# als244/ResNet

Hardware: AMD Instinct MI355X
Metric: images/sec ResNet-50 fp32 224x224 batch256 (higher is better)
Workload: dtype f32

## Files before the change

### resnet_amd/csrc/kernels_igemm.hip

```cpp
#include "mi_common.hpp"
#include <type_traits>
#include "mi_device.h"

typedef float f32x16 __attribute__((ext_vector_type(16)));
typedef float pf4 __attribute__((ext_vector_type(4)));

enum { IG_FWD = 0, IG_DGRAD = 1, IG_WGRAD = 2 };

struct IgArgs {
    int N, C, K, H, W, Ho, Wo;
    int HW, P;
    int ncols;
    int mtiles;
    int tiles;
    int ctiles;
    int klen;
    FastDiv fdP, fdWo, fdM;
    int full, tsplit, tklen, cpt;
    FastDiv fdTs, fdCpt;
    float *tailbuf;
    float *bn_part;
    int bn_np;
    const float *bnb_x, *bnb_mask, *bnb_mean;
    float *bnb_part;
// ... 345 lines not shown
        for (; it + 2 < ntiles; it++) kstep(Y, Y, it & 1);
        if (it + 1 < ntiles) { kstep(Y, NO, it & 1); it++; }
        if (it < ntiles) kstep(NO, NO, it & 1);
    }

    IG_T(2);
    if (MODE != IG_WGRAD && tail_id >= 0) {
        float *tb = g.tailbuf + (size_t)tail_id * (BM * 128);
#pragma unroll
        for (int j = 0; j < TN; j++)
#pragma unroll
            for (int i = 0; i < 2; i++)
#pragma unroll
                for (int r = 0; r < 16; r++)
                    tb[(wm * 64 + i * 32 + (r & 3) + 8 * (r >> 2) + 4 * (lane >> 5)) * 128 + wn * WNC + j * 32 + (lane & 31)] = acc[i][j][r];
        return;
    }
    if (MODE == IG_DGRAD && S == 1 && g.bnb_part) {
        constexpr int PPT = 4 / WMW;
        if ((g.P & 3) == 0) {
            constexpr int CPR = WNC / 4, RPI = 64 / CPR, PITCH = WNC + 4;
            float *img = ig_smem + wave * (32 * PITCH);
            const int c4 = (lane % CPR) * 4, r0 = lane / CPR;
            const int col = n0 + wn * WNC + c4;
            const bool cok = col < g.ncols;
            const uint32_t jc = cok ? (uint32_t)col : 0u;
            const uint32_t nimg = fd_div(jc, g.fdP);
            const size_t coff = (size_t)nimg * g.C * g.HW + (jc - nimg * g.P);
            const size_t pplane = (size_t)g.bnb_np * g.C;
#pragma unroll
            for (int i = 0; i < 2; i++) {
#pragma unroll
                for (int j = 0; j < TN; j++)
#pragma unroll
                    for (int r = 0; r < 16; r++)
                        img[((r & 3) + 8 * (r >> 2) + 4 * (lane >> 5)) * PITCH + j * 32 + (lane & 31)] = acc[i][j][r];
#pragma unroll
                for (int ps = 0; ps < 32 / RPI; ps++) {
                    const int rl = ps * RPI + r0;
                    const int row = m0 + wm * 64 + i * 32 + rl;
                    const size_t o = coff + (size_t)row * g.HW;
                    const pf4 z = {0.f, 0.f, 0.f, 0.f};
                    pf4 v = *(const pf4 *)(img + rl * PITCH + c4);
                    pf4 xv = z, mv = z;
                    if (cok) {
                        if (addend) v += *(const pf4 *)(addend + o);
                        xv = *(const pf4 *)(g.bnb_x + o);
                        mv = *(const pf4 *)(g.bnb_mask + o);
                    }
                    const float mean = g.bnb_mean[row];
                    float s1 = 0.f, s2 = 0.f;
#pragma unroll
                    for (int e = 0; e < 4; e++) {
                        v[e] = (cok && mv[e] > 0.f) ? v[e] : 0.f;
                        s1 += v[e];
                        s2 = fmaf(v[e], xv[e] - mean, s2);
                    }
                    if (cok) *(pf4 *)(Out + o) = v;
                    s1 += __int_as_float(__builtin_amdgcn_update_dpp(0, __float_as_int(s1), 0xB1, 0xF, 0xF, true));
                    s2 += __int_as_float(__builtin_amdgcn_update_dpp(0, __float_as_int(s2), 0xB1, 0xF, 0xF, true));
                    s1 += __int_as_float(__builtin_amdgcn_update_dpp(0, __float_as_int(s1), 0x4E, 0xF, 0xF, true));
                    s2 += __int_as_float(__builtin_amdgcn_update_dpp(0, __float_as_int(s2), 0x4E, 0xF, 0xF, true));
                    s1 += __int_as_float(__builtin_amdgcn_update_dpp(0, __float_as_int(s1), 0x141, 0xF, 0xF, true));
                    s2 += __int_as_float(__builtin_amdgcn_update_dpp(0, __float_as_int(s2), 0x141, 0xF, 0xF, true));
                    if (CPR == 16) {
                        s1 += __int_as_float(__builtin_amdgcn_update_dpp(0, __float_as_int(s1), 0x140, 0xF, 0xF, true));
                        s2 += __int_as_float(__builtin_amdgcn_update_dpp(0, __float_as_int(s2), 0x140, 0xF, 0xF, true));
                    }
                    if ((lane % CPR) == 0) {
                        const size_t po = (size_t)(ct * PPT + wn) * g.C + row;
                        g.bnb_part[po] = s1;
                        g.bnb_part[pplane + po] = s2;
                    }
                }
            }
            return;
        }
        size_t coffj[TN];
        bool cokj[TN];
#pragma unroll
        for (int j = 0; j < TN; j++) {
            const int col = n0 + wn * WNC + j * 32 + (lane & 31);
            cokj[j] = col < g.ncols;
            const uint32_t jc = cokj[j] ? (uint32_t)col : 0u;
            const uint32_t n = fd_div(jc, g.fdP);
            coffj[j] = (size_t)n * g.C * g.HW + (jc - n * g.P);
        }
        const size_t rstride = (size_t)g.HW;
        const size_t pplane = (size_t)g.bnb_np * g.C;
#pragma unroll
        for (int i = 0; i < 2; i++) {
            float s1[16], s2[16], mn[16];
#pragma unroll
            for (int r = 0; r < 16; r++) {
                s1[r] = 0.f; s2[r] = 0.f;
                mn[r] = g.bnb_mean[m0 + wm * 64 + i * 32 + (r & 3) + 8 * (r >> 2) + 4 * (lane >> 5)];
            }
#pragma unroll
            for (int j = 0; j < TN; j++) {
                float ad[16], xv[16], mv[16];
#pragma unroll
                for (int r = 0; r < 16; r++) {
                    const size_t o = coffj[j] + (size_t)(m0 + wm * 64 + i * 32 + (r & 3) + 8 * (r >> 2) + 4 * (lane >> 5)) * rstride;
                    ad[r] = (addend && cokj[j]) ? addend[o] : 0.f;
                    xv[r] = cokj[j] ? g.bnb_x[o] : 0.f;
                    mv[r] = cokj[j] ? g.bnb_mask[o] : 0.f;
                }
#pragma unroll
                for (int r = 0; r < 16; r++) {
                    const int row = m0 + wm * 64 + i * 32 + (r & 3) + 8 * (r >> 2) + 4 * (lane >> 5);
                    const float gv = mv[r] > 0.f ? acc[i][j][r] + ad[r] : 0.f;
                    if (cokj[j]) Out[coffj[j] + (size_t)row * rstride] = gv;
                    s1[r] += gv;
                    s2[r] = fmaf(gv, xv[r] - mn[r], s2[r]);
                }
            }
#pragma unroll
            for (int r = 0; r < 16; r++) {
                const float t1 = ig_half_sum32(s1[r]), t2 = ig_half_sum32(s2[r]);
                if ((lane & 31) == 31) {
                    const int row = m0 + wm * 64 + i * 32 + (r & 3) + 8 * (r >> 2) + 4 * (lane >> 5);
                    const size_t po = (size_t)(ct * PPT + wn) * g.C + row;
                    g.bnb_part[po] = t1;
                    g.bnb_part[pplane + po] = t2;
                }
            }
        }
        return;
    }
#pragma unroll
    for (int j = 0; j < TN; j++) {
        const int col = n0 + wn * WNC + j * 32 + (lane & 31);
        size_t coff, rstride;
        bool cok;
        if (MODE == IG_WGRAD) {
            const int lc = wn * WNC + j * 32 + (lane & 31);
            const int tap = CT64 ? wg_t + (lc >> 6) : wg_t;
            cok = tap < T;
            coff = ((size_t)((size_t)wg_split * T + tap) * g.K) * g.C + (CT64 ? (lc & 63) : cblk + lc);
            rstride = (size_t)g.C;
        } else {
            cok = col < g.ncols;
            const uint32_t jc = cok ? (uint32_t)col : 0u;
            const uint32_t n = fd_div(jc, g.fdP);
            const uint32_t p = jc - n * g.P;
            if (MODE == IG_FWD) { coff = (size_t)n * g.K * g.P + p; rstride = (size_t)g.P; }
            else if (S == 1) { coff = (size_t)n * g.C * g.HW + p; rstride = (size_t)g.HW; }
            else {
                const uint32_t a = fd_div(p, g.fdWo), b = p - a * g.Wo;
                coff = (size_t)n * g.C * g.HW + (size_t)(2 * a + ph) * g.W + 2 * b + pw;
                rstride = (size_t)g.HW;
            }
        }
        if (!cok) continue;
#pragma unroll
        for (int i = 0; i < 2; i++) {
            float ad[16];
            if (MODE == IG_DGRAD && addend) {
#pragma unroll
                for (int r = 0; r < 16; r++)
                    ad[r] = addend[coff + (size_t)(m0 + wm * 64 + i * 32 + (r & 3) + 8 * (r >> 2) + 4 * (lane >> 5)) * rstride];
            }
#pragma unroll
            for (int r = 0; r < 16; r++) {
                const int row = m0 + wm * 64 + i * 32 + (r & 3) + 8 * (r >> 2) + 4 * (lane >> 5);
                float v = acc[i][j][r];
                if (MODE == IG_DGRAD && addend) v += ad[r];
                Out[coff + (size_t)row * rstride] = v;
            }
        }
    }

    IG_T(3);
    if (MODE == IG_FWD && g.bn_part) {
        constexpr int PPT = 4 / WMW;
        float *tw = ig_smem + wave * (WNC * 64);
        const int l31 = lane & 31;
#pragma unroll
        for (int j = 0; j < TN; j++) {
            const int col = j * 32 + l31;
#pragma unroll
            for (int i = 0; i < 2; i++)
#pragma unroll
                for (int rg = 0; rg < 4; rg++) {
                    const int row4 = i * 8 + rg * 2 + (lane >> 5);
                    pf4 q4 = {acc[i][j][rg * 4 + 0], acc[i][j][rg * 4 + 1], acc[i][j][rg * 4 + 2], acc[i][j][rg * 4 + 3]};
                    *(pf4 *)(tw + col * 64 + ((row4 ^ (col & 15)) << 2)) = q4;
                }
        }
        const int nv = min(WNC, max(0, g.ncols - (n0 + wn * WNC)));
        const int row = lane;
        const float s0 = tw[(((row >> 2) ^ 0) << 2) + (row & 3)];
        float sd = 0.f, sq = 0.f;
#pragma unroll 8
        for (int c = 0; c < WNC; c++) {
            const float x = tw[c * 64 + ((((row >> 2) ^ (c & 15))) << 2) + (row & 3)];
            const float d = c < nv ? x - s0 : 0.f;
            sd += d;
            sq = fmaf(d, d, sq);
        }
        const float inv = nv > 0 ? 1.0f / (float)nv : 0.f;
        const size_t plane = (size_t)g.bn_np * g.K;
        const size_t o = (size_t)(ct * PPT + wn) * g.K + m0 + wm * 64 + row;
        g.bn_part[o] = (float)nv;
        g.bn_part[plane + o] = nv > 0 ? s0 + sd * inv : 0.f;
        g.bn_part[2 * plane + o] = fmaxf(sq - sd * sd * inv, 0.f);
    }
    IG_T(4);
}

template <int MODE, int BM>
__global__ void __launch_bounds__(256)
igemm_tail_reduce_kernel(float *__restrict__ Out, const float *__restrict__ addend, const IgArgs g) {
    const uint32_t L = (uint32_t)g.full + blockIdx.x;
    const uint32_t ct = fd_div(L, g.fdM);
    const int m0 = (int)(L - ct * g.mtiles) * BM;
    const int col = (int)ct * 128 + (threadIdx.x & 127);
    const bool cok = col < g.ncols;
    const uint32_t jc = cok ? (uint32_t)col : 0u;
    const uint32_t n = fd_div(jc, g.fdP);
    const uint32_t p = jc - n * g.P;
    size_t coff, rstride;
    if (MODE == IG_FWD) { coff = (size_t)n * g.K * g.P + p; rstride = (size_t)g.P; }
    else { coff = (size_t)n * g.C * g.HW + p; rstride = (size_t)g.HW; }
    const int row0 = (int)blockIdx.y * 16 + (int)(threadIdx.x >> 7) * 8;
    const float *tb = g.tailbuf + (size_t)blockIdx.x * g.tsplit * (BM * 128) + (size_t)row0 * 128 + (threadIdx.x & 127);
    float v[8];
#pragma unroll
    for (int i = 0; i < 8; i++) v[i] = 0.f;
    for (int z = 0; z < g.tsplit; z++) {
#pragma unroll
        for (int i = 0; i < 8; i++) v[i] += tb[(size_t)z * (BM * 128) + i * 128];
    }
    if (cok) {
#pragma unroll
        for (int i = 0; i < 8; i++) {
            const size_t o = coff + (size_t)(m0 + row0 + i) * rstride;
            float r = v[i];
            if (MODE == IG_DGRAD && addend) r += addend[o];
            Out[o] = r;
        }
    }
    if (MODE == IG_FWD && g.bn_part) {
        constexpr int PPT = BM == 128 ? 2 : 4;
        const int lane = threadIdx.x & 63, l31 = lane & 31;
        const int c32 = (int)ct * 128 + (int)(threadIdx.x & 127 & ~31);
        const int nv = min(32, max(0, g.ncols - c32));
        const size_t plane = (size_t)g.bn_np * g.K;
#pragma unroll
        for (int i = 0; i < 8; i++) {
            float mj, qj, nj = (float)nv;
            ig_half_stats(v[i], nv, l31, mj, qj);
            int pp = (int)(threadIdx.x & 127) >> 5;
            if (PPT == 2) {
                const float n2 = __shfl_xor(nj, 32, 64), m2o = __shfl_xor(mj, 32, 64), q2 = __shfl_xor(qj, 32, 64);
                if (lane == 0) ig_merge(nj, mj, qj, n2, m2o, q2);
                pp >>= 1;
            }
            if (PPT == 2 ? lane == 0 : l31 == 0) {
                const size_t o = (size_t)(ct * PPT + pp) * g.K + m0 + row0 + i;
                g.bn_part[o] = nj;
                g.bn_part[plane + o] = mj;
                g.bn_part[2 * plane + o] = qj;
            }
        }
    }
}

template <int T>
__global__ void __launch_bounds__(256)
igemm_wt_kernel(const float *__restrict__ w, float *__restrict__ out, int K, int C, int to_tck) {
    __shared__ float tile[32][T * 32 + 1];
    const int k0 = blockIdx.y * 32, c0 = blockIdx.x * 32;
    for (int e = threadIdx.x; e < 32 * T * 32; e += 256) {
        const int kr = e / (T * 32), x = e - kr * (T * 32);
        tile[kr][x] = w[((size_t)(k0 + kr) * C + c0) * T + x];
    }
    __syncthreads();
    for (int e = threadIdx.x; e < T * 32 * 32; e += 256) {
        const int t = e >> 10, u = (e >> 5) & 31, v = e & 31;
        if (to_tck) out[((size_t)t * C + c0 + u) * K + k0 + v] = tile[v][u * T + t];
        else out[((size_t)t * K + k0 + u) * C + c0 + v] = tile[u][v * T + t];
    }
}

__global__ void __launch_bounds__(256)
igemm_wt_all_kernel(const mid_wt_entry *__restrict__ entries, const int *__restrict__ tile_entry) {
    __shared__ float tile[32][9 * 32 + 1];
    const mid_wt_entry E = entries[tile_entry[blockIdx.x]];
    const int tl = (int)blockIdx.x - E.tile0, ctiles = E.C / 32, T = E.T;
    const int c0 = (tl % ctiles) * 32, k0 = (tl / ctiles) * 32, row = T * 32;
    for (int e = threadIdx.x; e < 32 * row; e += 256) {
        const int kr = e / row, x = e - kr * row;
        tile[kr][x] = E.w[((size_t)(k0 + kr) * E.C + c0) * T + x];
    }
    __syncthreads();
    for (int e = threadIdx.x; e < T * 1024; e += 256) {
        const int t = e >> 10, u = (e >> 5) & 31, v = e & 31;
        if (E.fwd) E.fwd[((size_t)t * E.C + c0 + u) * E.K + k0 + v] = tile[v][u * T + t];
        if (E.dgrad) E.dgrad[((size_t)t * E.K + k0 + u) * E.C + c0 + v] = tile[u][v * T + t];
    }
}

template <int T>
__global__ void __launch_bounds__(256)
igemm_wgrad_reduce_kernel(const float *__restrict__ part, float *__restrict__ dw, long KC, int splits) {
    const long i = (long)blockIdx.x * 256 + threadIdx.x;
    if (i >= KC) return;
    float s[T];
#pragma unroll
    for (int t = 0; t < T; t++) s[t] = 0.f;
    constexpr int U = T == 1 ? 8 : 2;
    int z = 0;
    for (; z + U <= splits; z += U) {
        float v[U][T];
#pragma unroll
        for (int u = 0; u < U; u++)
#pragma unroll
            for (int t = 0; t < T; t++) v[u][t] = part[((long)(z + u) * T + t) * KC + i];
#pragma unroll
        for (int u = 0; u < U; u++)
#pragma unroll
            for (int t = 0; t < T; t++) s[t] += v[u][t];
    }
    for (; z < splits; z++)
#pragma unroll
        for (int t = 0; t < T; t++) s[t] += part[((long)z * T + t) * KC + i];
#pragma unroll
    for (int t = 0; t < T; t++) dw[i * T + t] = s[t];
}

template <int T, int G>
__global__ void __launch_bounds__(256)
igemm_wgrad_reduce_g_kernel(const float *__restrict__ part, float *__restrict__ dw, long KC, int splits) {
    constexpr int OPB = 256 / G;
    __shared__ float sh[G][OPB][T];
    const int o = threadIdx.x % OPB, gq = threadIdx.x / OPB;
    const long i = (long)blockIdx.x * OPB + o;
    const int chunk = (splits + G - 1) / G, z0 = gq * chunk, z1 = min(splits, z0 + chunk);
    float s[T];
#pragma unroll
    for (int t = 0; t < T; t++) s[t] = 0.f;
    if (i < KC) {
        constexpr int U = T == 1 ? 8 : 2;
        int z = z0;
        for (; z + U <= z1; z += U) {
            float v[U][T];
#pragma unroll
            for (int u = 0; u < U; u++)
#pragma unroll
                for (int t = 0; t < T; t++) v[u][t] = part[((long)(z + u) * T + t) * KC + i];
#pragma unroll
            for (int u = 0; u < U; u++)
#pragma unroll
                for (int t = 0; t < T; t++) s[t] += v[u][t];
        }
        for (; z < z1; z++)
#pragma unroll
            for (int t = 0; t < T; t++) s[t] += part[((long)z * T + t) * KC + i];
    }
#pragma unroll
    for (int t = 0; t < T; t++) sh[gq][o][t] = s[t];
    __syncthreads();
    if (gq == 0 && i < KC) {
#pragma unroll
        for (int t = 0; t < T; t++) {
            float r = sh[0][o][t];
            for (int q = 1; q < G; q++) r += sh[q][o][t];
            dw[i * T + t] = r;
        }
    }
}
static bool igemm_wgrad_reduce_grouped(long KC, int splits) {
    static int on = -1;
    if (on < 0) { const char *e = getenv("RESNET_MI_WGRAD_REDUCE_G"); on = e ? atoi(e) : 1; }
    return on && splits >= 16 && mi_cdiv(KC, 256) < 1024;
}
static const char *igemm_wgrad_reduce_launch(hipStream_t st, const float *part, float *dw, long KC, int k, int splits) {
    const bool grouped = igemm_wgrad_reduce_grouped(KC, splits);
    if (k == 1) {
        if (grouped) hipLaunchKernelGGL((igemm_wgrad_reduce_g_kernel<1, 8>), dim3(mi_cdiv(KC, 32)), dim3(256), 0, st, part, dw, KC, splits);
        else hipLaunchKernelGGL(igemm_wgrad_reduce_kernel<1>, dim3(mi_cdiv(KC, 256)), dim3(256), 0, st, part, dw, KC, splits);
    } else {
        if (grouped) hipLaunchKernelGGL((igemm_wgrad_reduce_g_kernel<9, 8>), dim3(mi_cdiv(KC, 32)), dim3(256), 0, st, part, dw, KC, splits);
        else hipLaunchKernelGGL(igemm_wgrad_reduce_kernel<9>, dim3(mi_cdiv(KC, 256)), dim3(256), 0, st, part, dw, KC, splits);
    }
    return mi_trace_name("igemm_wgrad_reduce_kernel<k%d,%s>", k == 1 ? 1 : 3, grouped ? "grouped" : "flat");
}

__global__ void __launch_bounds__(256)
igemm_wgrad_reduce_t_kernel(const float *__restrict__ part, float *__restrict__ dw, int K, int C, int splits) {
    const long i = (long)blockIdx.x * 256 + threadIdx.x;
    if (i >= (long)K * C) return;
    float s = 0.f;
    int z = 0;
    for (; z + 8 <= splits; z += 8) {
        float v[8];
#pragma unroll
        for (int u = 0; u < 8; u++) v[u] = part[(long)(z + u) * K * C + i];
#pragma unroll
        for (int u = 0; u < 8; u++) s += v[u];
    }
    for (; z < splits; z++) s += part[(long)z * K * C + i];
    const int c = (int)(i / K), kk = (int)(i - (long)c * K);
    dw[(long)kk * C + c] = s;
}

enum { IGOP_FWD = 0, IGOP_DGRAD = 1, IGOP_WGRAD = 2 };
extern "C" int mi_igemm_supported(int op, int N, int C, int H, int K, int k, int stride) {
    if (!((k == 1 && stride == 1) || (k == 3 && (stride == 1 || stride == 2)))) return 0;
    if (H % stride || H / stride < 2) return 0;
    if ((double)N * C * H * H >= 1073741824.0 || (double)N * K * (H / stride) * (H / stride) >= 1073741824.0) return 0;
    if (op == IGOP_FWD) return C % 32 == 0 && K % 64 == 0;
    if (op == IGOP_DGRAD) return K % 32 == 0 && C % 64 == 0;
    if (C % 128 == 0 && K % 64 == 0) return 1;
    if (k == 3 && C == 64 && K % 64 == 0) return 1;
    return k == 1 && C % 64 == 0 && K % 128 == 0;
}
#define IG_SLOTS 512
#define IG_SLOTS64 768
static int igemm_wgrad_splits(int N, int C, int H, int K, int k, int stride) {
    const int bm = K % 128 == 0 ? 128 : 64;
    const long tiles = (C == 64 && k == 3 ? 5L : (long)k * k * (C / 128)) * (K / bm);
    const long ksteps = ((long)N * (H / stride) * (H / stride) + IG_BK - 1) / IG_BK;
    const long slots = bm == 128 ? IG_SLOTS : IG_SLOTS64;
    int best = 1;
    double best_eff = 0;
    for (int s = 1; s <= 512; s++) {
        if (s > 1 && ksteps / s < 48) break;
        const double waves = (double)tiles * s / slots;
        const double eff = waves / (double)((long)((tiles * s + slots - 1) / slots));
        if (eff > best_eff + 0.02) { best_eff = eff; best = s; }
    }
    return best;
}
static bool igemm_wgrad_swapped(int C, int K, int k) { return k == 1 && C % 128 != 0; }
extern "C" size_t mi_igemm_part_floats(int N, int C, int H, int K, int k, int stride) {
    if (igemm_wgrad_swapped(C, K, k)) return (size_t)igemm_wgrad_splits(N, K, H, C, k, stride) * K * C;
    return (size_t)igemm_wgrad_splits(N, C, H, K, k, stride) * k * k * K * C;
}

#define IG_TAIL_FLOATS ((size_t)IG_SLOTS * 128 * 128)
extern "C" size_t mi_igemm_tail_floats(void) { return IG_TAIL_FLOATS; }
static void igemm_tail_plan(IgArgs &g, int ksteps, float *tailbuf, int bm) {
    const int slots = bm == 128 ? IG_SLOTS : IG_SLOTS64;
    g.full = g.tiles; g.tsplit = 1; g.tklen = ksteps; g.tailbuf = tailbuf;
    g.fdTs = make_fastdiv(1);
    static int on = -1;
    if (on < 0) { const char *e = getenv("RESNET_MI_IGEMM_TAIL"); on = e ? atoi(e) : 1; }
    if (!on || !tailbuf) return;
    const int rem = g.tiles % slots;
    if (rem == 0) return;
    if (rem * 2 > slots) return;
    int s = slots / rem;
    if (s > 16) s = 16;
    while (s > 1 && ksteps / s < 8) s--;
    if (s < 2) return;
    g.tklen = (ksteps + s - 1) / s;
    g.tsplit = (ksteps + g.tklen - 1) / g.tklen;
    g.full = g.tiles - rem;
    g.fdTs = make_fastdiv(g.tsplit);
}

static int igemm_pick_bm(int M, int coltiles, int ksteps, int k) {
    if (M % 128) return 64;
    double best = 0;
    int pick = 128;
    for (int bm = 128; bm >= 64; bm -= 64) {
        const long B = (long)(M / bm) * coltiles;
        const long slots = bm == 128 ? IG_SLOTS : IG_SLOTS64;
        const long rem = B % slots;
        double tail = 0;
        if (rem) {
            int s = (int)(slots / rem);
            if (s > 16) s = 16;
            while (s > 1 && ksteps / s < 8) s--;
            tail = rem * 2 > slots || s < 2 ? 1.0 : 1.0 / s + 0.03;
        }
        const double t = ((double)(B / slots) + tail) * (bm == 128 ? 1.0 : k == 1 ? 0.70 : 0.80);
        if (bm == 128 || t < best * 0.97) { if (bm == 128 || t < best) { best = t; pick = bm; } }
    }
    static int force = -1;
    if (force < 0) { const char *e = getenv("RESNET_MI_IGEMM_BM"); force = e ? atoi(e) : 0; }
    if (force == 64 || (force == 128 && M % 128 == 0)) return force;
    return pick;
}

static void igemm_geometry(IgArgs &g, int N, int C, int H, int K, int stride) {
    g.N = N; g.C = C; g.K = K; g.H = H; g.W = H; g.Ho = H / stride; g.Wo = H / stride;
    g.HW = H * H; g.P = g.Ho * g.Wo;
    g.ncols = N * g.P;
    g.fdP = make_fastdiv(g.P); g.fdWo = make_fastdiv(g.Wo);
}
static int igemm_plan_tiles(IgArgs &g, int op, int N, int C, int H, int K, int k, int stride) {
    igemm_geometry(g, N, C, H, K, stride);
    const int M = op == IGOP_FWD ? K : C, red = op == IGOP_FWD ? C : K;
    const int bm = (op == IGOP_FWD || stride == 1) ? igemm_pick_bm(M, mi_cdiv(g.ncols, 128), k * k * (red / IG_BK), k) : (M % 128 == 0 ? 128 : 64);
    g.mtiles = M / bm;
    g.tiles = g.mtiles * mi_cdiv(g.ncols, 128);
    g.fdM = make_fastdiv(g.mtiles);
    g.cpt = red / IG_BK; g.fdCpt = make_fastdiv(g.cpt);
    return bm;
}
static int igemm_plan_wgrad(IgArgs &g, int N, int C, int H, int K, int k, int stride, bool swapped, int *used) {
    int bm;
    if (swapped) {
        const int splits = igemm_wgrad_splits(N, K, H, C, 1, 1);
        igemm_geometry(g, N,  K, H,  C, 1);
        bm = C % 128 == 0 ? 128 : 64;
        g.mtiles = C / bm;
        g.ctiles = K / 128;
        g.tiles = g.mtiles * g.ctiles;
        g.klen = mi_cdiv(mi_cdiv(N * g.P, splits), IG_BK) * IG_BK;
    } else {
        const int T = k * k;
        const int splits = igemm_wgrad_splits(N, C, H, K, k, stride);
        igemm_geometry(g, N, C, H, K, stride);
        bm = K % 128 == 0 ? 128 : 64;
        g.mtiles = K / bm;
        g.ctiles = C / 128;
        g.tiles = C == 64 ? g.mtiles * ((T + 1) / 2) : g.mtiles * T * g.ctiles;
        g.klen = mi_cdiv(mi_cdiv(N * g.P, splits), IG_BK) * IG_BK;
    }
    g.fdM = make_fastdiv(g.mtiles);
    g.full = g.tiles; g.tsplit = 1; g.fdTs = make_fastdiv(1); g.cpt = 1; g.fdCpt = make_fastdiv(1);
    *used = mi_cdiv(N * g.P, g.klen);
    return bm;
}
static thread_local const char *ig_variant = "igemm_kernel";
template <int MODE, int KS, int S, int WMW, bool VB = false>
static int igemm_launch_t(hipStream_t st, dim3 grid, const float *A, const float *B, float *out, const float *addend, const IgArgs &g) {
    constexpr int BM = 64 * WMW;
    constexpr int LDA = (MODE == IG_WGRAD) ? BM + 1 : BM + 4, LDB = (MODE == IG_WGRAD) ? 129 : 132;
    constexpr size_t lds = (size_t)2 * IG_BK * (LDA + LDB) * sizeof(float);
    static int attr_set = 0;
    if (!attr_set) {
        if (lds > 64 * 1024 &&
            hipFuncSetAttribute((const void *)igemm_kernel<MODE, KS, S, WMW, VB>, hipFuncAttributeMaxDynamicSharedMemorySize, (int)lds) != hipSuccess) {
            mi_record_error("igemm_kernel", "cannot raise the dynamic LDS limit");
            return -1;
        }
        attr_set = 1;
    }
    hipLaunchKernelGGL((igemm_kernel<MODE, KS, S, WMW, VB>), grid, dim3(256), lds, st, A, B, out, addend, g);
    ig_variant = mi_trace_name("igemm_kernel<%s,k%d,s%d,bm%d%s%s>", MODE == IG_FWD ? "fwd" : MODE == IG_DGRAD ? "dgrad" : "wgrad", KS, S, BM, VB ? ",vb" : "",
                               g.tsplit > 1 ? ",tail" : "");
    return 0;
}
template <int MODE>
static int igemm_launch(hipStream_t st, dim3 grid, const float *A, const float *B, float *out, const float *addend, const IgArgs &g,
                        int k, int stride, int bm) {
#define IGL(KS_, S_)                                                                                      \
    if (k == KS_ && stride == S_)                                                                         \
        return bm == 128 ? igemm_launch_t<MODE, KS_, S_, 2>(st, grid, A, B, out, addend, g)               \
                         : igemm_launch_t<MODE, KS_, S_, 1>(st, grid, A, B, out, addend, g);
    if (MODE != IG_WGRAD && k == 1 && stride == 1 && g.P % 4 == 0)
        return bm == 128 ? igemm_launch_t<MODE, 1, 1, 2, true>(st, grid, A, B, out, addend, g)
                         : igemm_launch_t<MODE, 1, 1, 1, true>(st, grid, A, B, out, addend, g);
    if (MODE == IG_WGRAD && k == 3 && g.C == 64) {
        if (stride == 1) return bm == 128 ? igemm_launch_t<MODE, 3, 1, 2, true>(st, grid, A, B, out, addend, g) : igemm_launch_t<MODE, 3, 1, 1, true>(st, grid, A, B, out, addend, g);
        return bm == 128 ? igemm_launch_t<MODE, 3, 2, 2, true>(st, grid, A, B, out, addend, g) : igemm_launch_t<MODE, 3, 2, 1, true>(st, grid, A, B, out, addend, g);
    }
    IGL(1, 1) IGL(3, 1) IGL(3, 2)
#undef IGL
    return -2;
}
static int igemm_fam(int k) { return k == 1 ? MI_FAM_GEMM : MI_FAM_PCONV; }

extern "C" int mi_igemm_fwd(mid_stream s, mid_workspace *ws, const float *x, const float *w, float *y, int N, int C, int H, int K, int k,
                            int stride, mid_bn_parts *parts) {
    hipStream_t st = (hipStream_t)s;
    const int T = k * k;
    if (parts) parts->nparts = 0;
    if (!mi_igemm_supported(IGOP_FWD, N, C, H, K, k, stride)) { mi_record_error("mi_igemm_fwd", "shape not supported by the implicit GEMM"); return -2; }
    if (!ws || ws->wt_floats < (size_t)T * C * K) { mi_record_error("mi_igemm_fwd", "workspace too small"); return -3; }
    const float *A = ws->pre_fwd;
    if (!A) {
        if (k == 1) hipLaunchKernelGGL(igemm_wt_kernel<1>, dim3(C / 32, K / 32), dim3(256), 0, st, w, ws->wt, K, C, 1);
        else hipLaunchKernelGGL(igemm_wt_kernel<9>, dim3(C / 32, K / 32), dim3(256), 0, st, w, ws->wt, K, C, 1);
        MI_LAUNCH_CHECK("igemm_wt_kernel");
        A = ws->wt;
    }
    IgArgs g = {};
    const int bm = igemm_plan_tiles(g, IGOP_FWD, N, C, H, K, k, stride);
    igemm_tail_plan(g, T * g.cpt, ws->wt_floats >= (size_t)T * C * K + IG_TAIL_FLOATS ? ws->wt + (size_t)T * C * K : nullptr, bm);
    if (parts) {
        parts->nparts = 0;
        const int np = mi_cdiv(g.ncols, 128) * (bm == 128 ? 2 : 4);
        if (parts->buf && parts->floats >= (size_t)3 * np * K) { g.bn_part = parts->buf; g.bn_np = np; parts->nparts = np; }
    }
    mi_prof_begin(st, igemm_fam(k), 2.0 * T * (double)g.ncols * C * K,
                  4.0 * ((double)N * C * g.HW + (double)T * C * K + (double)g.ncols * K));
    int rc = igemm_launch<IG_FWD>(st, dim3(g.full + (g.tiles - g.full) * g.tsplit), A, x, y, nullptr, g, k, stride, bm);
    if (!rc && g.tsplit > 1) {
        if (bm == 128) hipLaunchKernelGGL((igemm_tail_reduce_kernel<IG_FWD, 128>), dim3(g.tiles - g.full, 8), dim3(256), 0, st, y, nullptr, g);
        else hipLaunchKernelGGL((igemm_tail_reduce_kernel<IG_FWD, 64>), dim3(g.tiles - g.full, 4), dim3(256), 0, st, y, nullptr, g);
    }
    mi_prof_end(st);
    if (rc) return rc;
    MI_LAUNCH_CHECK(ig_variant);
    return 0;
}

extern "C" int mi_igemm_dgrad(mid_stream s, mid_workspace *ws, const float *w, const float *dy, float *dx, const float *addend, int N,
                              int C, int H, int K, int k, int stride, mid_bn_bwd_parts *fz) {
    hipStream_t st = (hipStream_t)s;
    if (fz) fz->nparts = 0;
    if (!mi_igemm_supported(IGOP_DGRAD, N, C, H, K, k, stride)) { mi_record_error("mi_igemm_dgrad", "shape not supported by the implicit GEMM"); return -2; }
    const int T = k * k;
    const float *A = w;
    if (k == 3) {
        if (!ws || ws->wt_floats < (size_t)T * C * K) { mi_record_error("mi_igemm_dgrad", "workspace too small"); return -3; }
        if (ws->pre_dgrad) A = ws->pre_dgrad;
        else {
            hipLaunchKernelGGL(igemm_wt_kernel<9>, dim3(C / 32, K / 32), dim3(256), 0, st, w, ws->wt, K, C, 0);
            MI_LAUNCH_CHECK("igemm_wt_kernel");
            A = ws->wt;
        }
    }
    IgArgs g = {};
    const int bm = igemm_plan_tiles(g, IGOP_DGRAD, N, C, H, K, k, stride);
    bool fused = false;
    if (fz && fz->buf && stride == 1) {
        const int np = mi_cdiv(g.ncols, 128) * (bm == 128 ? 2 : 4);
        if (fz->floats >= (size_t)2 * np * C) {
            g.bnb_x = (const float *)fz->x; g.bnb_mask = (const float *)fz->mask; g.bnb_mean = fz->means;
            g.bnb_part = fz->buf; g.bnb_np = np; fz->nparts = np;
            fused = true;
        }
    }
    igemm_tail_plan(g, T * g.cpt, !fused && stride == 1 && ws && ws->wt_floats >= (size_t)T * C * K + IG_TAIL_FLOATS ? ws->wt + (size_t)T * C * K : nullptr, bm);
    mi_prof_begin(st, igemm_fam(k), 2.0 * T * (double)g.ncols * C * K,
                  4.0 * ((double)g.ncols * K + (double)T * C * K + (double)N * C * g.HW * ((addend ? 2 : 1) + (fused ? 2 : 0))));
    int rc = igemm_launch<IG_DGRAD>(st, dim3(g.full + (g.tiles - g.full) * g.tsplit, stride == 2 ? 4 : 1), A, dy, dx, addend, g, k, stride, bm);
    if (!rc && g.tsplit > 1) {
        if (bm == 128) hipLaunchKernelGGL((igemm_tail_reduce_kernel<IG_DGRAD, 128>), dim3(g.tiles - g.full, 8), dim3(256), 0, st, dx, addend, g);
        else hipLaunchKernelGGL((igemm_tail_reduce_kernel<IG_DGRAD, 64>), dim3(g.tiles - g.full, 4), dim3(256), 0, st, dx, addend, g);
    }
    mi_prof_end(st);
    if (rc) return rc;
    MI_LAUNCH_CHECK(ig_variant);
    return 0;
}

extern "C" int mi_igemm_wgrad(mid_stream s, mid_workspace *ws, const float *x, const float *dy, float *dw, int N, int C, int H, int K, int k,
                              int stride) {
    hipStream_t st = (hipStream_t)s;
    if (!mi_igemm_supported(IGOP_WGRAD, N, C, H, K, k, stride)) { mi_record_error("mi_igemm_wgrad", "shape not supported by the implicit GEMM"); return -2; }
    if (igemm_wgrad_swapped(C, K, k)) {
        const int splits = igemm_wgrad_splits(N, K, H, C, 1, 1);
        if (!ws || ws->part_floats < (size_t)splits * K * C) { mi_record_error("mi_igemm_wgrad", "workspace too small"); return -3; }
        IgArgs g = {};
        int used;
        const int bm = igemm_plan_wgrad(g, N, C, H, K, k, stride, true, &used);
        const int kd = N * g.P;
        mi_prof_begin(st, igemm_fam(1), 2.0 * (double)kd * C * K, 4.0 * ((double)N * C * g.HW + (double)kd * K + (double)C * K));
        const int rc = igemm_launch<IG_WGRAD>(st, dim3(g.tiles, used),  x,  dy, ws->part, nullptr, g, 1, 1, bm);
        mi_prof_end(st);
        if (rc) return rc;
        MI_LAUNCH_CHECK_V("%s,transposed", ig_variant);
        hipLaunchKernelGGL(igemm_wgrad_reduce_t_kernel, dim3(mi_cdiv((long)K * C, 256)), dim3(256), 0, st, ws->part, dw, K, C, used);
        MI_LAUNCH_CHECK("igemm_wgrad_reduce_t_kernel");
        return 0;
    }
    const int T = k * k;
    const int splits = igemm_wgrad_splits(N, C, H, K, k, stride);
    if (!ws || ws->part_floats < (size_t)splits * T * K * C) { mi_record_error("mi_igemm_wgrad", "workspace too small"); return -3; }
    IgArgs g = {};
    int used;
    const int bm = igemm_plan_wgrad(g, N, C, H, K, k, stride, false, &used);
    const int kd = N * g.P;
    mi_prof_begin(st, igemm_fam(k), 2.0 * T * (double)kd * C * K,
                  4.0 * ((double)N * C * g.HW + (double)kd * K + (double)T * C * K));
    const int rc = igemm_launch<IG_WGRAD>(st, dim3(g.tiles, used), dy, x, ws->part, nullptr, g, k, stride, bm);
    mi_prof_end(st);
    if (rc) return rc;
    MI_LAUNCH_CHECK(ig_variant);
    const long KC = (long)K * C;
    MI_LAUNCH_CHECK(igemm_wgrad_reduce_launch(st, ws->part, dw, KC, k, used));
    return 0;
}

int mi_igemm_wgrad_reduce(hipStream_t st, const float *part, float *dw, int K, int C, int k, int splits) {
    const long KC = (long)K * C;
    MI_LAUNCH_CHECK(igemm_wgrad_reduce_launch(st, part, dw, KC, k, splits));
    return 0;
}

#ifdef IG_STAMP
extern "C" int mi_debug_igemm_stamps(unsigned long long *dst, int nblocks) {
    return hipMemcpyFromSymbol(dst, HIP_SYMBOL(ig_stamps), sizeof(unsigned long long) * 8 * (size_t)nblocks) == hipSuccess ? 0 : -1;
}
#endif

extern "C" int mid_igemm_plan(int op, int N, int C, int H, int K, int k, int stride, int out[9]) {
    for (int i = 0; i < 9; i++) out[i] = 0;
    if (!mi_igemm_supported(op, N, C, H, K, k, stride)) return 0;
    out[0] = 1;
    IgArgs g = {};
    if (op == IGOP_WGRAD) {
        int used;
        out[1] = igemm_plan_wgrad(g, N, C, H, K, k, stride, igemm_wgrad_swapped(C, K, k), &used);
        out[2] = g.tiles; out[3] = g.tiles; out[4] = 1; out[5] = g.klen / IG_BK; out[6] = used; out[7] = g.tiles; out[8] = mi_cdiv(N * g.P, IG_BK);
        return 1;
    }
    const int bm = igemm_plan_tiles(g, op, N, C, H, K, k, stride);
    float dummy;
    igemm_tail_plan(g, k * k * g.cpt, (op == IGOP_FWD || stride == 1) ? &dummy : nullptr, bm);
    out[1] = bm; out[2] = g.tiles; out[3] = g.full; out[4] = g.tsplit; out[5] = g.tklen; out[6] = 1;
    out[7] = g.full + (g.tiles - g.full) * g.tsplit; out[8] = k * k * g.cpt;
    return 1;
}
extern "C" int mid_wgrad_reduce_grouped(int K, int C, int splits) { return igemm_wgrad_reduce_grouped((long)K * C, splits) ? 1 : 0; }
extern "C" int mid_igemm_conv_plan(int op, int N, int C, int H, int K, int k, int stride, int out[7]) {
    int o[9];
    if (!mid_igemm_plan(op, N, C, H, K, k, stride, o)) return 0;
    out[0] = o[1]; out[1] = 128; out[2] = o[2]; out[3] = o[3]; out[4] = o[4]; out[5] = o[6];
    out[6] = op == IGOP_WGRAD && !igemm_wgrad_swapped(C, K, k) ? mid_wgrad_reduce_grouped(K, C, o[6]) : 0;
    return 1;
}

extern "C" int mid_conv_prelayout_all(mid_stream s, const mid_wt_entry *entries_dev, const int *tile_entry_dev, int ntiles) {
    if (ntiles <= 0) return 0;
    hipLaunchKernelGGL(igemm_wt_all_kernel, dim3(ntiles), dim3(256), 0, (hipStream_t)s, entries_dev, tile_entry_dev);
    MI_LAUNCH_CHECK("igemm_wt_all_kernel");
    return 0;
}
```

Baseline: 2461.

## Vectorize wgrad split-K reduction kernels with float4 loads and LDS-staged coalesced stores

Rewrites the weight-gradient split-K reduction kernels to load and accumulate float4 vectors instead of scalars. For 3x3 kernels, results are staged through shared memory so the stores to dw are coalesced. The transposed reduce kernel is restructured to stage split slices through LDS and transpose a KxC tile before writing. This adds alignment and divisibility checks that return errors for unsupported shapes, and the grouped path uses smaller blocks.

Result: no change. 2462, median of 4 (+0.1%).

```diff
diff --git a/resnet_amd/csrc/kernels_igemm.hip b/resnet_amd/csrc/kernels_igemm.hip
--- a/resnet_amd/csrc/kernels_igemm.hip
+++ b/resnet_amd/csrc/kernels_igemm.hip
@@ -671,18 +671,19 @@
     }
 }
 
+
 template <int T>
 __global__ void __launch_bounds__(256)
-igemm_wgrad_reduce_kernel(const float *__restrict__ part, float *__restrict__ dw, long KC, int splits) {
-    const long i = (long)blockIdx.x * 256 + threadIdx.x;
-    if (i >= KC) return;
-    float s[T];
+igemm_wgrad_reduce_kernel(const pf4 *__restrict__ part, pf4 *__restrict__ dw, long KC, int splits) {
+    __shared__ pf4 sh[T == 1 ? 1 : 256 * T];
+    const long i = min((long)blockIdx.x * blockDim.x + threadIdx.x, KC - 1);
+    pf4 s[T];
 #pragma unroll
     for (int t = 0; t < T; t++) s[t] = 0.f;
-    constexpr int U = T == 1 ? 8 : 2;
+    constexpr int U = T == 1 ? 8 : 4;
     int z = 0;
     for (; z + U <= splits; z += U) {
-        float v[U][T];
+        pf4 v[U][T];
 #pragma unroll
         for (int u = 0; u < U; u++)
 #pragma unroll
@@ -692,87 +693,140 @@
 #pragma unroll
             for (int t = 0; t < T; t++) s[t] += v[u][t];
     }
+#pragma unroll 4
     for (; z < splits; z++)
 #pragma unroll
         for (int t = 0; t < T; t++) s[t] += part[((long)z * T + t) * KC + i];
-#pragma unroll
-    for (int t = 0; t < T; t++) dw[i * T + t] = s[t];
-}
-
+    if (T == 1) {
+        if ((long)blockIdx.x * blockDim.x + threadIdx.x < KC) dw[i] = s[0];
+        return;
+    }
+    float *mine = (float *)&sh[threadIdx.x * T];
+#pragma unroll
+    for (int j = 0; j < 4; j++)
+#pragma unroll
+        for (int t = 0; t < T; t++) mine[j * T + t] = s[t][j];
+    __syncthreads();
+    const long run0 = (long)blockIdx.x * blockDim.x * T;
+    for (int e = threadIdx.x; e < (int)blockDim.x * T; e += blockDim.x)
+        if (run0 + e < KC * T) dw[run0 + e] = sh[e];
+}
+
+#define IGR_COLS(T) ((T) == 1 ? 16 : 8)
 template <int T, int G>
-__global__ void __launch_bounds__(256)
-igemm_wgrad_reduce_g_kernel(const float *__restrict__ part, float *__restrict__ dw, long KC, int splits) {
-    constexpr int OPB = 256 / G;
-    __shared__ float sh[G][OPB][T];
-    const int o = threadIdx.x % OPB, gq = threadIdx.x / OPB;
-    const long i = (long)blockIdx.x * OPB + o;
+__global__ void __launch_bounds__(G * IGR_COLS(T))
+igemm_wgrad_reduce_g_kernel(const pf4 *__restrict__ part, pf4 *__restrict__ dw, long KC, int splits) {
+    constexpr int COLS = IGR_COLS(T);
+    __shared__ pf4 sh[G][COLS][T];
+    __shared__ pf4 run[T == 1 ? 1 : COLS * T];
+    const int o = threadIdx.x % COLS, gq = threadIdx.x / COLS;
+    const long col = (long)blockIdx.x * COLS + o, i = min(col, KC - 1);
     const int chunk = (splits + G - 1) / G, z0 = gq * chunk, z1 = min(splits, z0 + chunk);
-    float s[T];
+    pf4 s[T];
 #pragma unroll
     for (int t = 0; t < T; t++) s[t] = 0.f;
-    if (i < KC) {
-        constexpr int U = T == 1 ? 8 : 2;
-        int z = z0;
-        for (; z + U <= z1; z += U) {
-            float v[U][T];
-#pragma unroll
-            for (int u = 0; u < U; u++)
-#pragma unroll
-                for (int t = 0; t < T; t++) v[u][t] = part[((long)(z + u) * T + t) * KC + i];
-#pragma unroll
-            for (int u = 0; u < U; u++)
-#pragma unroll
-                for (int t = 0; t < T; t++) s[t] += v[u][t];
-        }
-        for (; z < z1; z++)
-#pragma unroll
-            for (int t = 0; t < T; t++) s[t] += part[((long)z * T + t) * KC + i];
+    constexpr int U = T == 1 ? 16 : 4;
+    for (int z = z0; z < z1; z += U) {
+        const int n = z1 - z;
+        pf4 v[U][T];
+#pragma unroll
+        for (int u = 0; u < U; u++)
+#pragma unroll
+            for (int t = 0; t < T; t++) v[u][t] = part[((long)(z + min(u, n - 1)) * T + t) * KC + i];
+#pragma unroll
+        for (int u = 0; u < U; u++)
+#pragma unroll
+            for (int t = 0; t < T; t++) s[t] += u < n ? v[u][t] : pf4(0.f);
     }
 #pragma unroll
     for (int t = 0; t < T; t++) sh[gq][o][t] = s[t];
     __syncthreads();
-    if (gq == 0 && i < KC) {
+    if (gq == 0) {
+        float *mine = (float *)&run[T == 1 ? 0 : o * T];
 #pragma unroll
         for (int t = 0; t < T; t++) {
-            float r = sh[0][o][t];
+            pf4 r = sh[0][o][t];
             for (int q = 1; q < G; q++) r += sh[q][o][t];
-            dw[i * T + t] = r;
-        }
-    }
+            if (T == 1) { if (col < KC) dw[col] = r; }
+            else
+#pragma unroll
+                for (int j = 0; j < 4; j++) mine[j * T + t] = r[j];
+        }
+    }
+    if (T == 1) return;
+    __syncthreads();
+    const long run0 = (long)blockIdx.x * COLS * T;
+    for (int e = threadIdx.x; e < COLS * T; e += G * COLS)
+        if (run0 + e < KC * T) dw[run0 + e] = run[e];
 }
 static bool igemm_wgrad_reduce_grouped(long KC, int splits) {
     static int on = -1;
     if (on < 0) { const char *e = getenv("RESNET_MI_WGRAD_REDUCE_G"); on = e ? atoi(e) : 1; }
     return on && splits >= 16 && mi_cdiv(KC, 256) < 1024;
 }
+static bool igemm_wgrad_reduce_vec_ok(const float *part, const float *dw, long KC) {
+    if (KC > 0 && KC % 4 == 0 && ((uintptr_t)part | (uintptr_t)dw) % 16 == 0) return true;
+    mi_record_error("igemm_wgrad_reduce", "K*C is not a multiple of 4 or a buffer is not 16-byte aligned");
+    return false;
+}
 static const char *igemm_wgrad_reduce_launch(hipStream_t st, const float *part, float *dw, long KC, int k, int splits) {
     const bool grouped = igemm_wgrad_reduce_grouped(KC, splits);
+    const pf4 *p4 = (const pf4 *)part;
+    pf4 *d4 = (pf4 *)dw;
+    const long KC4 = KC / 4;
+    const int fb = KC4 < 256 * 256 ? 64 : 256;
     if (k == 1) {
-        if (grouped) hipLaunchKernelGGL((igemm_wgrad_reduce_g_kernel<1, 8>), dim3(mi_cdiv(KC, 32)), dim3(256), 0, st, part, dw, KC, splits);
-        else hipLaunchKernelGGL(igemm_wgrad_reduce_kernel<1>, dim3(mi_cdiv(KC, 256)), dim3(256), 0, st, part, dw, KC, splits);
+        if (grouped) hipLaunchKernelGGL((igemm_wgrad_reduce_g_kernel<1, 8>), dim3(mi_cdiv(KC4, IGR_COLS(1))), dim3(8 * IGR_COLS(1)), 0, st, p4, d4, KC4, splits);
+        else hipLaunchKernelGGL(igemm_wgrad_reduce_kernel<1>, dim3(mi_cdiv(KC4, fb)), dim3(fb), 0, st, p4, d4, KC4, splits);
     } else {
-        if (grouped) hipLaunchKernelGGL((igemm_wgrad_reduce_g_kernel<9, 8>), dim3(mi_cdiv(KC, 32)), dim3(256), 0, st, part, dw, KC, splits);
-        else hipLaunchKernelGGL(igemm_wgrad_reduce_kernel<9>, dim3(mi_cdiv(KC, 256)), dim3(256), 0, st, part, dw, KC, splits);
+        if (grouped) hipLaunchKernelGGL((igemm_wgrad_reduce_g_kernel<9, 8>), dim3(mi_cdiv(KC4, IGR_COLS(9))), dim3(8 * IGR_COLS(9)), 0, st, p4, d4, KC4, splits);
+        else hipLaunchKernelGGL(igemm_wgrad_reduce_kernel<9>, dim3(mi_cdiv(KC4, fb)), dim3(fb), 0, st, p4, d4, KC4, splits);
     }
     return mi_trace_name("igemm_wgrad_reduce_kernel<k%d,%s>", k == 1 ? 1 : 3, grouped ? "grouped" : "flat");
 }
 
+#define IGT_C 4
+#define IGT_K 32
+#define IGT_COLS (IGT_C * IGT_K / 4)
+#define IGT_LG (256 / IGT_COLS)
+#define IGT_U 12
+#define IGT_TURN (IGT_LG * IGT_U)
 __global__ void __launch_bounds__(256)
-igemm_wgrad_reduce_t_kernel(const float *__restrict__ part, float *__restrict__ dw, int K, int C, int splits) {
-    const long i = (long)blockIdx.x * 256 + threadIdx.x;
-    if (i >= (long)K * C) return;
+igemm_wgrad_reduce_t_kernel(const pf4 *__restrict__ part, float *__restrict__ dw, int K, int C, int splits) {
+    __shared__ pf4 st[IGT_TURN][IGT_COLS];
+    __shared__ float tile[IGT_K][IGT_C + 1];
+    const int kt = K / IGT_K, c0 = ((int)blockIdx.x / kt) * IGT_C, k0 = ((int)blockIdx.x % kt) * IGT_K;
+    const int col = threadIdx.x % IGT_COLS, lg = threadIdx.x / IGT_COLS;
+    const int cr = col / (IGT_K / 4), kq = col % (IGT_K / 4);
+    const long plane = (long)K * C / 4, i = ((long)(c0 + cr) * K + k0) / 4 + kq;
+    pf4 v[IGT_U];
+#pragma unroll
+    for (int u = 0; u < IGT_U; u++) v[u] = part[(long)min(lg * IGT_U + u, splits - 1) * plane + i];
     float s = 0.f;
-    int z = 0;
-    for (; z + 8 <= splits; z += 8) {
-        float v[8];
-#pragma unroll
-        for (int u = 0; u < 8; u++) v[u] = part[(long)(z + u) * K * C + i];
-#pragma unroll
-        for (int u = 0; u < 8; u++) s += v[u];
-    }
-    for (; z < splits; z++) s += part[(long)z * K * C + i];
-    const int c = (int)(i / K), kk = (int)(i - (long)c * K);
-    dw[(long)kk * C + c] = s;
+    for (int z = 0; z < splits; z += IGT_TURN) {
+#pragma unroll
+        for (int u = 0; u < IGT_U; u++) st[lg * IGT_U + u][col] = v[u];
+        __syncthreads();
+        if (z + IGT_TURN < splits) {
+#pragma unroll
+            for (int u = 0; u < IGT_U; u++) v[u] = part[(long)min(z + IGT_TURN + lg * IGT_U + u, splits - 1) * plane + i];
+        }
+        if (threadIdx.x < 4 * IGT_COLS) {
+            const float *p = (const float *)&st[0][0] + threadIdx.x;
+            const int n = min(IGT_TURN, splits - z);
+#pragma unroll 8
+            for (int q = 0; q < n; q++) s += p[q * 4 * IGT_COLS];
+        }
+        __syncthreads();
+    }
+    if (threadIdx.x < 4 * IGT_COLS) tile[threadIdx.x % IGT_K][threadIdx.x / IGT_K] = s;
+    __syncthreads();
+    if (threadIdx.x < IGT_K) {
+        pf4 r;
+#pragma unroll
+        for (int j = 0; j < 4; j++) r[j] = tile[threadIdx.x][j];
+        *(pf4 *)&dw[(long)(k0 + threadIdx.x) * C + c0] = r;
+    }
 }
 
 enum { IGOP_FWD = 0, IGOP_DGRAD = 1, IGOP_WGRAD = 2 };
@@ -1028,7 +1082,8 @@
         mi_prof_end(st);
         if (rc) return rc;
         MI_LAUNCH_CHECK_V("%s,transposed", ig_variant);
-        hipLaunchKernelGGL(igemm_wgrad_reduce_t_kernel, dim3(mi_cdiv((long)K * C, 256)), dim3(256), 0, st, ws->part, dw, K, C, used);
+        if (K % IGT_K || C % IGT_C || !igemm_wgrad_reduce_vec_ok(ws->part, dw, (long)K * C)) return -2;
+        hipLaunchKernelGGL(igemm_wgrad_reduce_t_kernel, dim3((K / IGT_K) * (C / IGT_C)), dim3(256), 0, st, (const pf4 *)ws->part, dw, K, C, used);
         MI_LAUNCH_CHECK("igemm_wgrad_reduce_t_kernel");
         return 0;
     }
@@ -1046,12 +1101,14 @@
     if (rc) return rc;
     MI_LAUNCH_CHECK(ig_variant);
     const long KC = (long)K * C;
+    if (!igemm_wgrad_reduce_vec_ok(ws->part, dw, KC)) return -2;
     MI_LAUNCH_CHECK(igemm_wgrad_reduce_launch(st, ws->part, dw, KC, k, used));
     return 0;
 }
 
 int mi_igemm_wgrad_reduce(hipStream_t st, const float *part, float *dw, int K, int C, int k, int splits) {
     const long KC = (long)K * C;
+    if (!igemm_wgrad_reduce_vec_ok(part, dw, KC)) return -2;
     MI_LAUNCH_CHECK(igemm_wgrad_reduce_launch(st, part, dw, KC, k, splits));
     return 0;
 }
```
